# dashpay/agora-blsful

Hardware: NVIDIA B200
Metric: verified sigs/sec, 1M-batch G2Impl (higher is better)
Workload: dtype u32 limbs (381-bit modular integers)

## Files before the change

### agora-blsful_b200/csrc/blsgpu.cu

```cuda
#include <cuda_runtime.h>
#include <nvtx3/nvToolsExt.h>
#include <sys/random.h>

#include <algorithm>
#include <atomic>
#include <functional>
#include <cstdio>
#include <cstdlib>
#include <cstring>
#include <memory>
#include <mutex>
#include <string>
#include <unordered_map>
#include <thread>
#include <vector>

#include "../../include/blsgpu.h"
#include "kernels.cuh"

using namespace bls;

namespace {

thread_local std::string g_create_error;
// ... 347 lines not shown
  bool use_rlc = true, use_msm = false;
  int rbits = 0;
  std::vector<Level> lv;
  const PkA* d_pk = nullptr;
  const SigA *d_sig = nullptr, *d_h = nullptr;
  uint8_t* d_status = nullptr;
  Fp12* d_F = nullptr;
  SigJ *d_S = nullptr, *d_Sitem = nullptr, *d_msm_root = nullptr;
  RlcScalar* d_r = nullptr;
  Digest* d_root = nullptr;
  uint8_t* d_ok = nullptr;
  uint32_t* d_idx = nullptr;
  PkA* x_pk = nullptr;
  SigA* x_h = nullptr;
  uint8_t* x_pre = nullptr;
  M6Arg* x_args = nullptr;
  SLineRec* x_lines = nullptr;
  Fp12* x_T = nullptr;
  size_t x_cap = 0;
  M6Arg* big_args = nullptr;
  SLineRec* big_lines = nullptr;
  size_t big_items = 0;
  bool root_T_ready = false;
  const Fp12* rootF() const { return d_F + lv.back().off; }
  const SigJ* rootS() const { return use_msm ? d_msm_root : use_rlc ? d_S + lv.back().off : d_S; }
  bool big_rounds(size_t count) const { return count > PROBE_SMALL && big_items >= 6 * PROBE_SMALL; }
  size_t round_size(size_t count) const { return big_rounds(count) ? std::min(x_cap, big_items / 6) : PROBE_SMALL; }
};

size_t probe_cap(size_t leaves) { return std::max<size_t>(PROBE_SMALL, std::min<size_t>(leaves, 4096) + 16); }
template <class PkA, class SigA, class A>
void take_probe_scratch(A& a, Pipe<PkA, SigA>& P, size_t cap) {
  const size_t small = std::min(cap, PROBE_SMALL);
  P.x_cap = cap;
  P.d_ok = a.template take<uint8_t>(cap);
  P.d_idx = a.template take<uint32_t>(cap);
  P.x_pk = a.template take<PkA>(6 * cap);
  P.x_h = a.template take<SigA>(6 * cap);
  P.x_pre = a.template take<uint8_t>(6 * cap);
  P.x_T = a.template take<Fp12>(cap);
  P.x_args = a.template take<M6Arg>(6 * small);
  P.x_lines = a.template take<SLineRec>(6 * small * M6_LINE_RECS);
}
template <class PkA, class SigA>
size_t probe_scratch_bytes(size_t cap) {
  ArenaSize a;
  Pipe<PkA, SigA> P;
  take_probe_scratch(a, P, cap);
  return a.off;
}
template <class PkA, class SigA>
int set_probe_smem(blsgpu_ctx* ctx) {
  CK(cudaFuncSetAttribute(k_m6_lines<PkA, SigA>, cudaFuncAttributeMaxDynamicSharedMemorySize, M6_LINES_SMEM));
  CK(cudaFuncSetAttribute(k_m6_accum, cudaFuncAttributeMaxDynamicSharedMemorySize, M6_ACCUM_SMEM));
  CK(cudaFuncSetAttribute(k_final6, cudaFuncAttributeMaxDynamicSharedMemorySize, FE6_SMEM));
  return BLSGPU_OK;
}

template <class J>
int reduce_levels(blsgpu_ctx* ctx, const std::vector<Level>& lv, size_t first, Fp12* F, J* S) {
  for (size_t k = first; k + 1 < lv.size(); k++) {
    if (F) REDUCE_FP12(lv[k].cnt, (const Fp12*)(F + lv[k].off), lv[k + 1].cnt, F + lv[k + 1].off);
    if (S) REDUCE_JAC(J, lv[k].cnt, (const J*)(S + lv[k].off), lv[k + 1].cnt, S + lv[k + 1].off);
  }
  return BLSGPU_OK;
}

int seg_reduce(blsgpu_ctx* ctx, size_t n_out, const uint32_t* off, const Fp12* in, Fp12* out) {
  if (n_out <= REDUCE_WIDE_MAX)
    LAUNCH(k_seg_reduce_fp12_w, blocks_for(n_out * 16), TPB, n_out, off, in, out);
  else
    LAUNCH(k_seg_reduce_fp12, blocks_for(n_out), TPB, n_out, off, in, out);
  return BLSGPU_OK;
}
template <class J>
int seg_reduce(blsgpu_ctx* ctx, size_t n_out, const uint32_t* off, const J* in, J* out) {
  if (n_out <= REDUCE_WIDE_MAX)
    LAUNCH((k_seg_reduce_jac_w<J>), blocks_for(n_out * 16), TPB, n_out, off, in, out);
  else
    LAUNCH((k_seg_reduce_jac<J>), blocks_for(n_out), TPB, n_out, off, in, out);
  return BLSGPU_OK;
}
template <class T>
int seg_reduce_levels(blsgpu_ctx* ctx, const SegLevels& s, const uint32_t* d_off, T* nodes, T* top) {
  size_t in_off = 0, out_off = s.n[0], o = 0;
  for (size_t k = 1; k < s.n.size(); k++) {
    const size_t n_out = s.n[k];
    CKR(seg_reduce(ctx, n_out, d_off + o, (const T*)(nodes + in_off), k + 1 == s.n.size() ? top : nodes + out_off));
    o += n_out + 1;
    in_off = out_off;
    out_off += n_out;
  }
  return BLSGPU_OK;
}

int digest_root(blsgpu_ctx* ctx, size_t leaves, Digest* d_dig, Digest* d_root) {
  const std::vector<Level> ld = make_levels(leaves);
  for (size_t k = 0; k + 1 < ld.size(); k++)
    LAUNCH(k_digest_reduce, blocks_for(ld[k + 1].cnt), TPB, ld[k].cnt, d_dig + ld[k].off, ld[k + 1].cnt, d_dig + ld[k + 1].off);
  CK(cudaMemcpyAsync(d_root, d_dig + ld.back().off, sizeof(Digest), cudaMemcpyDeviceToDevice, ctx->stream));
  CK(cudaMemcpyAsync(d_root + 1, ctx->salt, 32, cudaMemcpyHostToDevice, ctx->stream));
  return BLSGPU_OK;
}

template <class PkA, class SigA>
int probe_miller(blsgpu_ctx* ctx, Pipe<PkA, SigA>& P, cudaStream_t stream, size_t cnt, M6Arg* args, SLineRec* lines) {
// ... 3160 lines not shown
```

### agora-blsful_b200/csrc/kernels.cuh

```cuda
#pragma once
#include <cuda_runtime.h>

#include "h2c.cuh"
#include "pairing.cuh"
#include "miller6.cuh"
#include "finalexp6.cuh"
#include "fr.cuh"

namespace bls {

template <class A>
struct PtInfo;
template <>
struct PtInfo<G1Aff> {
  static const int LEN = 48;
  typedef G1Jac Jac;
  typedef Fp F;
};
template <>
struct PtInfo<G2Aff> {
  static const int LEN = 96;
  typedef G2Jac Jac;
  typedef Fp2 F;
};
// ... 251 lines not shown
  size_t j = BLS_TID();
  if (j >= n_out) return;
  Sha256 s;
  sha256_init(s);
  for (int m = 0; m < 16; m++) {
    size_t idx = j + (size_t)m * n_out;
    if (idx < n_in) sha256_update(s, in[idx].b, 32);
  }
  Digest d;
  sha256_final(s, d.b);
  out[j] = d;
}
constexpr int RLC_MAX_WORDS = 4;
__device__ __forceinline__ void rlc_scalar(uint32_t k[RLC_MAX_WORDS], const Digest* root, size_t i, int rbits) {
  Sha256 s;
  sha256_init(s);
  sha256_update(s, root[0].b, 32);
  sha256_update(s, root[1].b, 32);
  uint8_t ib[8];
  for (int b = 0; b < 8; b++) ib[b] = (uint8_t)((uint64_t)i >> (8 * b));
  sha256_update(s, ib, 8);
  uint8_t d[32];
  sha256_final(s, d);
  uint32_t any = 0;
#pragma unroll
  for (int w = 0; w < RLC_MAX_WORDS; w++) {
    const uint32_t v = (uint32_t)d[4 * w] | ((uint32_t)d[4 * w + 1] << 8) | ((uint32_t)d[4 * w + 2] << 16) | ((uint32_t)d[4 * w + 3] << 24);
    k[w] = 32 * w < rbits ? v : 0u;
    any |= k[w];
  }
  if (any == 0) k[0] = 1;
}

__device__ __forceinline__ void miller_item(Fp12& f, const G1Aff& pk, const G2Aff& h, const uint32_t* k, bool scale) {
  MillerG1 mp;
  if (scale) {
    G1Jac pj;
    jac_mul_aff(pj, pk, k, 2);
    miller_prepare(mp, pj);
  } else {
    miller_prepare(mp, pk);
  }
  miller_loop(f, mp, h);
}
__device__ __forceinline__ void miller_item(Fp12& f, const G2Aff& pk, const G1Aff& h, const uint32_t* k, bool scale) {
  miller_item(f, h, pk, k, scale);
}
constexpr int M6_LINES_TPB = 128;
constexpr int M6_LINES_PAIRS = M6_LINES_TPB / 2;
constexpr int M6_LINES_SMEM = M6_NREG * M6_LINES_PAIRS * (int)sizeof(SFp2);
constexpr int M6_ITEMS_PER_BLOCK = 120;
constexpr int M6_ACCUM_SMEM = 4 * 30 * (int)sizeof(SAccRec);
constexpr size_t M6_LINE_RECS = (size_t)M6_STEPS * 3;

__device__ __forceinline__ const G1Aff& m6_g1(const G1Aff* pk, const G2Aff* h, size_t i) { return pk[i]; }
__device__ __forceinline__ const G1Aff& m6_g1(const G2Aff* pk, const G1Aff* h, size_t i) { return h[i]; }
__device__ __forceinline__ const G2Aff& m6_g2(const G1Aff* pk, const G2Aff* h, size_t i) { return h[i]; }
__device__ __forceinline__ const G2Aff& m6_g2(const G2Aff* pk, const G1Aff* h, size_t i) { return pk[i]; }

template <class PkA, class HA>
__global__ void __launch_bounds__(128, BLS_MIN_BLOCKS) k_m6_prep(size_t n, size_t base, const PkA* __restrict__ pk, const HA* __restrict__ h,
                                                 const uint8_t* __restrict__ pre, const Digest* __restrict__ root, int rbits,
                                                 M6Arg* __restrict__ args) {
  size_t c = BLS_TID();
  if (c >= n) return;
  const size_t i = base + c;
  if (pre[i] != ST_OK) return;
  G1Aff p = m6_g1(pk, h, i);
  MillerG1 mp;
  if (rbits) {
    uint32_t sc[RLC_MAX_WORDS];
    rlc_scalar(sc, root, i, rbits);
    G1Jac pj;
    jac_mul_aff_w4(pj, p, sc, rbits / 4);
    miller_prepare(mp, pj);
  } else {
    miller_prepare(mp, p);
  }
  M6Arg a;
  const G2Aff q = m6_g2(pk, h, i);
  m6_make_arg(a, mp, q);
  args[c] = a;
}

template <class PkA, class HA>
__global__ void __launch_bounds__(M6_LINES_TPB, 3) k_m6_lines(size_t n, size_t base, const M6Arg* __restrict__ args, const PkA* __restrict__ pk,
                                                             const HA* __restrict__ h, const uint8_t* __restrict__ pre, SLineRec* __restrict__ lines) {
  extern __shared__ __align__(16) uint8_t m6_smem[];
  const int hh = threadIdx.x & 1, pib = threadIdx.x >> 1;
  const size_t c = (size_t)blockIdx.x * M6_LINES_PAIRS + pib;
  const bool active = c < n && pre[base + (c < n ? c : 0)] == ST_OK;
  const size_t cc = active ? c : 0;
  const G2Aff& q = m6_g2(pk, h, base + cc);
  SopSpaces cx = m6_spaces_line(reinterpret_cast<SFp2*>(m6_smem) + pib, M6_LINES_PAIRS, args + cc, lines + cc * M6_LINE_RECS);
  if (active && hh == 0) {
    const G2Aff qv = q;
    m6_init_point(cx, qv);
  }
  __syncwarp();
  const uint64_t e = K_X_ABS;
#pragma unroll 1
  for (int i = 62; i >= 0; i--) {
#pragma unroll 1
    for (int pass = 0; pass < 1 + (int)((e >> i) & 1); pass++) {
      const M6Op* prog = pass == 0 ? K_M6_DBL : K_M6_ADD;
      const int nops = pass == 0 ? K_M6_DBL_N : K_M6_ADD_N;
#pragma unroll 1
      for (int o = 0; o < nops; o++) {
        const M6Op* op = prog + o;
        int32_t res[NL], other[NL];
        double vb = 0;
        if (active) vb = m6_op_compute(res, op, cx, hh);
        if (op->dst >= SOPX_LINE) {
#pragma unroll
          for (int j = 0; j < NL; j++) other[j] = __shfl_xor_sync(0xffffffffu, res[j], 1);
        }
        __syncwarp();
        if (active) m6_op_store(op, cx, hh, res, other, vb);
        __syncwarp();
      }
      cx.line += 3;
    }
  }
}

#ifndef M6_ACC_BLOCKS
#define M6_ACC_BLOCKS 3
#endif
__global__ void __launch_bounds__(128, M6_ACC_BLOCKS) k_m6_accum(size_t n, size_t base, const uint8_t* __restrict__ pre, const SLineRec* __restrict__ lines,
                                                     Fp12* __restrict__ out) {
  extern __shared__ __align__(16) uint8_t m6_smem[];
  const int warp = threadIdx.x >> 5, lane = threadIdx.x & 31;
  const int g = lane / 6, k = lane - 6 * g;
  const bool lane_on = g < 5;
  SAccRec* F = reinterpret_cast<SAccRec*>(m6_smem) + warp * 30 + 6 * (lane_on ? g : 0);
  const unsigned gsync = lane_on ? 63u << (6 * g) : 0xc0000000u;
  const size_t group = ((size_t)blockIdx.x * 4 + warp) * 5 + g;
  const size_t item = group * 6 + k;
  const bool active = lane_on && item < n && pre[base + item] == ST_OK;
  const unsigned ball = __ballot_sync(0xffffffffu, active);
  const unsigned gmask = lane_on ? (ball >> (6 * g)) & 63u : 0u;
  if (lane_on) {
    SFp2 init;
    if (k == 0) sfp2_one(init); else sfp2_zero(init);
    sacc_from_sfp2(F[k], init);
  }
  __syncwarp();
  const SLineRec* gl = lines + group * 6 * M6_LINE_RECS;
  const uint64_t e = K_X_ABS;
  int step = 0;
  if (gmask != 0) {
#pragma unroll 1
    for (int i = 62; i >= 0; i--) {
      if (i != 62) m6_sqr_lane(F + k, F, k, gsync);
      const int nst = 1 + (int)((e >> i) & 1);
#pragma unroll 1
      for (int st = 0; st < nst; st++, step++) {
#pragma unroll 1
        for (int j = 0; j < 6; j++) {
          {
            const int jn = j == 5 ? 0 : j + 1;
            const int sn = j == 5 ? step + 1 : step;
            if (k < 3 && sn < M6_STEPS) {
              const SLineRec* nx = gl + (size_t)jn * M6_LINE_RECS + 3 * sn + k;
              asm volatile("prefetch.global.L1 [%0];" ::"l"(nx));
              asm volatile("prefetch.global.L1 [%0];" ::"l"(reinterpret_cast<const uint8_t*>(nx) + 128));
            }
          }
          if ((gmask >> j) & 1u) m6_mul_line_lane(F + k, F, gl + (size_t)j * M6_LINE_RECS + 3 * step, k, gsync);
        }
      }
    }
  }
  __syncwarp();
  if (lane_on && group * 6 < n) m6_finish_lane(*fp12_coeff(out[base / 6 + group], k), F[k], k);
}

template <class SigA>
__global__ void __launch_bounds__(128, BLS_MIN_BLOCKS) k_scale_sig(size_t n, const SigA* __restrict__ sig, const uint8_t* __restrict__ pre,
                                                   const Digest* __restrict__ root, int rbits,
                                                   typename PtInfo<SigA>::Jac* __restrict__ out) {
  size_t i = BLS_TID();
  if (i >= n) return;
  typename PtInfo<SigA>::Jac s;
  if (pre[i] != ST_OK) {
    jac_set_inf(s);
  } else {
    uint32_t k[RLC_MAX_WORDS];
    rlc_scalar(k, root, i, rbits);
    SigA a = sig[i];
    jac_mul_aff(s, a, k, rbits / 32);
  }
  out[i] = s;
}

constexpr int MSM_CHUNK = 16;
struct RlcScalar {
  uint64_t lo, hi;
};
__device__ __forceinline__ uint32_t msm_digit(const RlcScalar& r, int c, int w) {
  const int bit = c * w;
  const uint64_t v = bit >= 64 ? r.hi >> (bit - 64) : bit == 0 ? r.lo : (r.lo >> bit) | (r.hi << (64 - bit));
  return (uint32_t)v & ((1u << c) - 1u);
}
__global__ void __launch_bounds__(128) k_msm_count(size_t n, const uint8_t* __restrict__ pre, const Digest* __restrict__ root, int rbits, int c,
                                                   int nwin, RlcScalar* __restrict__ r_out, uint32_t* __restrict__ counts) {
  size_t i = BLS_TID();
  if (i >= n) return;
  RlcScalar r = {0, 0};
  if (pre[i] == ST_OK) {
    uint32_t k[RLC_MAX_WORDS];
    rlc_scalar(k, root, i, rbits);
    r.lo = (uint64_t)k[0] | ((uint64_t)k[1] << 32);
    r.hi = (uint64_t)k[2] | ((uint64_t)k[3] << 32);
  }
  r_out[i] = r;
  for (int w = 0; w < nwin; w++) {
    const uint32_t d = msm_digit(r, c, w);
    if (d) atomicAdd(&counts[((size_t)w << c) + d], 1u);
  }
}
__global__ void __launch_bounds__(1024) k_msm_scan(int c, const uint32_t* __restrict__ counts, uint32_t* __restrict__ offsets,
                                                   uint32_t* __restrict__ cursor) {
// ... 1112 lines not shown
```

### agora-blsful_b200/csrc/miller6.cuh

```cuda
#pragma once
#include "pairing.cuh"
#include "sfp.cuh"

namespace bls {

constexpr int M6_GROUP = 6;

#define M6_S(ia, ib, xi, sh) {SOPX_F + ia, SOPX_F + ib, sh, 0, (xi) ? SOP_XI : 0, 0, 0, 0}
BLS_CONST SopTerm K_M6_SQR[6][4] = {
    {M6_S(0, 0, 0, 0), M6_S(1, 5, 1, 1), M6_S(2, 4, 1, 1), M6_S(3, 3, 1, 0)},
    {M6_S(0, 1, 0, 1), M6_S(2, 5, 1, 1), M6_S(3, 4, 1, 0), M6_S(3, 4, 1, 0)},
    {M6_S(0, 2, 0, 1), M6_S(1, 1, 0, 0), M6_S(3, 5, 1, 1), M6_S(4, 4, 1, 0)},
    {M6_S(0, 3, 0, 1), M6_S(1, 2, 0, 1), M6_S(4, 5, 1, 0), M6_S(4, 5, 1, 0)},
    {M6_S(0, 4, 0, 1), M6_S(1, 3, 0, 1), M6_S(2, 2, 0, 0), M6_S(5, 5, 1, 0)},
    {M6_S(0, 5, 0, 1), M6_S(1, 4, 0, 1), M6_S(2, 3, 0, 0), M6_S(2, 3, 0, 0)},
};
#undef M6_S
BLS_CONST SopTerm K_M6_MUL_LINE[3] = {
    {SOPX_FREL + 0, SOPX_JL + 0, 0, 0, 0, 0, 0, 0},
    {SOPX_FREL + 2, SOPX_JL + 1, 0, 0, SOP_XI_LT2, 0, 0, 0},
    {SOPX_FREL + 3, SOPX_JL + 2, 0, 0, SOP_XI_LT3, 0, 0, 0},
};

BLS_HD void m6_sqr_lane(SAccRec* out, const SAccRec* F, int k, unsigned sync_mask) { sopw(out, K_M6_SQR[k], 4, F, nullptr, k, sync_mask); }
BLS_HD void m6_mul_line_lane(SAccRec* out, const SAccRec* F, const SLineRec* line, int k, unsigned sync_mask) {
  sopw(out, K_M6_MUL_LINE, 3, F, line, k, sync_mask);
}

BLS_HD Fp2* fp12_coeff(Fp12& f, int k) {
  Fp6& h = (k & 1) ? f.c1 : f.c0;
  return (k >> 1) == 0 ? &h.c0 : (k >> 1) == 1 ? &h.c1 : &h.c2;
}

BLS_HD void m6_finish_lane(Fp2& out, const SAccRec& fa, int k) {
  SFp2 fk, t;
  sfp2_from_sacc(fk, fa);
  t = fk;
  if (k & 1) sfp2_neg(t, fk);
  Fp2 u;
  fp2_from_sfp2(u, t);
  fred(out, u);
}

enum : uint8_t {
  RX = 0, RY, RZ, RT0, RT1, RT2, RT3, RT4, RT5, RT6,
  M6_NREG,
  RPX = SOPX_P, RNPY = SOPX_P + 1, RPZ = SOPX_P + 2,
  RNQX = SOPX_P + 3, RQY = SOPX_P + 4,
  RL0 = SOPX_LINE, RL2 = SOPX_LINE + 1, RL3 = SOPX_LINE + 2,
  RNONE = SOPX_NONE
};
struct M6Op {
  uint8_t kind;
  uint8_t dst, nt, fp;
  SopTerm t[3];
  int8_t lx, ly, lz;
  uint8_t xr, yr, zr, lfl, pad;
};
#define M6_T(a, b) {a, b, 0, 0, 0, 0, 0, 0}
#define M6_TS(a, sha, b, shb, fl) {a, b, sha, shb, fl, 0, 0, 0}
#define M6_SQ(a) {a, a, 0, 0, SOP_SQR, 0, 0, 0}
#define M6_SQS(a, sha, shb, fl) {a, a, sha, shb, (fl) | SOP_SQR, 0, 0, 0}
#define M6_SOP1(dst, t0) {0, dst, 1, 0, {t0, t0, t0}, 0, 0, 0, RNONE, RNONE, RNONE, 0, 0}
#define M6_SOP2(dst, t0, t1) {0, dst, 2, 0, {t0, t1, t1}, 0, 0, 0, RNONE, RNONE, RNONE, 0, 0}
#define M6_SOP3(dst, t0, t1, t2) {0, dst, 3, 0, {t0, t1, t2}, 0, 0, 0, RNONE, RNONE, RNONE, 0, 0}
#define M6_SOPFP(dst, t0) {0, dst, 1, 1, {t0, t0, t0}, 0, 0, 0, RNONE, RNONE, RNONE, 0, 0}
#define M6_SOPFP2(dst, t0, t1) {0, dst, 2, 1, {t0, t1, t1}, 0, 0, 0, RNONE, RNONE, RNONE, 0, 0}
#define M6_LIN(dst, x, lx, fl, y, ly, z, lz) {1, dst, 0, 0, {M6_T(RNONE, RNONE), M6_T(RNONE, RNONE), M6_T(RNONE, RNONE)}, lx, ly, lz, x, y, z, fl, 0}
BLS_CONST M6Op K_M6_DBL[] = {
    M6_SOP1(RT0, M6_SQ(RY)),
    M6_SOP1(RT1, M6_SQ(RZ)),
    M6_SOP1(RT2, M6_SQ(RX)),
    M6_SOP1(RT3, M6_T(RX, RY)),
    M6_SOP1(RT4, M6_T(RY, RZ)),
    M6_LIN(RT1, RT1, 12, SOP_XI, RNONE, 0, RNONE, 0),
    M6_LIN(RT5, RT1, -3, 0, RT0, 1, RNONE, 0),
    M6_LIN(RT6, RT1, 3, 0, RT0, 1, RNONE, 0),
    M6_LIN(RT2, RT2, 3, 0, RNONE, 0, RNONE, 0),
    M6_SOP1(RX, M6_TS(RT3, 1, RT5, 0, 0)),
    M6_LIN(RT5, RT1, 1, 0, RT0, -1, RNONE, 0),
    M6_SOPFP(RL0, M6_T(RT5, RPZ)),
    M6_LIN(RT1, RT1, 2, 0, RNONE, 0, RNONE, 0),
    M6_SOP3(RY, M6_SQ(RT6), M6_SQS(RT1, 1, 0, SOP_NEG), M6_SQS(RT1, 0, 0, SOP_NEG)),
    M6_SOP1(RZ, M6_TS(RT0, 2, RT4, 1, 0)),
    M6_SOPFP(RL2, M6_T(RT2, RPX)),
    M6_SOPFP(RL3, M6_TS(RT4, 1, RNPY, 0, 0)),
};
BLS_CONST M6Op K_M6_ADD[] = {
    M6_SOP1(RT0, M6_T(RQY, RZ)),
    M6_SOP1(RT1, M6_TS(RNQX, 0, RZ, 0, SOP_NEG)),
    M6_LIN(RT0, RT0, 1, 0, RY, -1, RNONE, 0),
    M6_LIN(RT1, RT1, 1, 0, RX, -1, RNONE, 0),
    M6_SOP1(RT2, M6_SQ(RT1)),
    M6_SOP1(RT3, M6_T(RT1, RT2)),
    M6_SOP1(RT4, M6_T(RT2, RX)),
    M6_SOP2(RT2, M6_T(RT1, RQY), M6_T(RT0, RNQX)),
    M6_SOPFP(RL0, M6_T(RT2, RPZ)),
    M6_SOPFP(RL2, M6_T(RT0, RPX)),
    M6_SOPFP(RL3, M6_T(RT1, RNPY)),
    M6_SOP1(RT2, M6_SQ(RT0)),
    M6_SOP1(RT2, M6_T(RT2, RZ)),
    M6_LIN(RT2, RT2, 1, 0, RT3, -1, RT4, -2),
    M6_SOP1(RX, M6_T(RT1, RT2)),
    M6_SOP3(RY, M6_T(RT0, RT4), M6_TS(RT0, 0, RT2, 0, SOP_NEG), M6_TS(RT3, 0, RY, 0, SOP_NEG)),
    M6_SOP1(RZ, M6_T(RT3, RZ)),
};
#undef M6_T
#undef M6_TS
#undef M6_SQ
#undef M6_SQS
#undef M6_SOP1
#undef M6_SOP2
#undef M6_SOP3
#undef M6_SOPFP
#undef M6_SOPFP2
#undef M6_LIN
constexpr int K_M6_DBL_N = (int)(sizeof(K_M6_DBL) / sizeof(M6Op));
constexpr int K_M6_ADD_N = (int)(sizeof(K_M6_ADD) / sizeof(M6Op));

BLS_FN void m6_run(const M6Op* prog, int n, const SopSpaces& cx) {
#pragma unroll 1
  for (int i = 0; i < n; i++) {
    const M6Op* op = prog + i;
    const bool to_line = op->dst >= SOPX_LINE;
    SFp2* dst = to_line ? nullptr : sop_rec(cx, op->dst);
    if (op->kind == 0) {
      sop2f(dst, to_line ? cx.line + (op->dst - SOPX_LINE) : nullptr, op->t, op->nt, op->fp, cx);
    } else {
      sfp2_lin(*dst, sop_rec(cx, op->xr), op->lx, op->lfl, op->yr == RNONE ? nullptr : sop_rec(cx, op->yr), op->ly,
               op->zr == RNONE ? nullptr : sop_rec(cx, op->zr), op->lz);
    }
  }
}

BLS_HD double m6_op_compute(int32_t* res, const M6Op* op, const SopSpaces& cx, int h) {
  if (op->kind == 0) return sop1_compute(res, op->t, op->nt, op->fp, cx, h);
  return sfp2_lin_half(res, sop_rec(cx, op->xr), op->lx, op->lfl, op->yr == RNONE ? nullptr : sop_rec(cx, op->yr), op->ly,
                       op->zr == RNONE ? nullptr : sop_rec(cx, op->zr), op->lz, h);
}
// ... 39 lines not shown
```

### agora-blsful_b200/csrc/sfp.cuh

```cuda
#pragma once
#include "fp2.cuh"

#if !defined(SOP_KARATSUBA)
#define SOP_KARATSUBA 1
#endif

namespace bls {

struct alignas(16) SFp2 {
  int32_t w[2 * NL];
#if defined(BLS_TRACK)
  double vb;
  double lb;
#endif
};

struct alignas(16) SLineRec {
  int32_t w[48];
#if defined(BLS_TRACK)
  double vb, lb;
#endif
};
struct alignas(16) SAccRec {
  int32_t w[64];
// ... 98 lines not shown
    sb[i] = alu_add_s32(b[i], b[H + i]);
  }
#pragma unroll
  for (int i = 0; i < H; i++) {
#pragma unroll
    for (int j = 0; j < H; j++) T[H + i + j] += (uint64_t)((int64_t)sa[i] * (int64_t)sb[j]);
  }
#else
#pragma unroll
  for (int i = 0; i < NL; i++) {
#pragma unroll
    for (int j = 0; j < NL; j++) T[i + j] += (uint64_t)((int64_t)a[i] * (int64_t)b[j]);
  }
#endif
}

BLS_HD void sop_redc(int32_t* out, uint64_t* T) {
#pragma unroll
  for (int i = 0; i < NL; i++) {
    const uint32_t m = opaque32(((uint32_t)T[i] * K_PINV28) & M28);
#pragma unroll
    for (int j = 0; j < NL; j++) T[i + j] += (uint64_t)m * p28(j);
    T[i + 1] += (uint64_t)((int64_t)T[i] >> 28);
  }
  int64_t c = 0;
#pragma unroll
  for (int j = 0; j < NL - 1; j++) {
    c += (int64_t)T[NL + j];
    const int64_t t = c + (1 << 27);
    out[j] = (int32_t)((uint32_t)t & M28) - (1 << 27);
    c = t >> 28;
  }
  out[NL - 1] = (int32_t)(c + (int64_t)T[2 * NL - 1]);
}

struct alignas(16) SopKeep {
  uint64_t v[2 * NL];
};
BLS_HD void sop_keep_st(SopKeep& k, int i, uint64_t a, uint64_t b) {
#if defined(__CUDA_ARCH__)
  asm volatile("st.local.v2.u64 [%0], {%1, %2};" ::"l"(__cvta_generic_to_local(&k.v[2 * i])), "l"(a), "l"(b) : "memory");
#else
  k.v[2 * i] = a;
  k.v[2 * i + 1] = b;
#endif
}
BLS_HD void sop_keep_ld(const SopKeep& k, int i, uint64_t& a, uint64_t& b) {
#if defined(__CUDA_ARCH__)
  asm volatile("ld.local.v2.u64 {%0, %1}, [%2];" : "=l"(a), "=l"(b) : "l"(__cvta_generic_to_local(&k.v[2 * i])) : "memory");
#else
  a = k.v[2 * i];
  b = k.v[2 * i + 1];
#endif
}

struct SopPrep {
  int32_t m0, m1, n1, ng, sh;
};
BLS_HD SopPrep sop_prep(int half, int xi, int neg, int sh) {
  SopPrep p;
  const int p0 = half == 0, p1 = half == 1, p2 = half == 2;
  p.m0 = -((p1 ^ 1) | xi);
  p.m1 = -(((p2 & xi) ^ 1) & ((p0 & (xi ^ 1)) ^ 1));
  p.n1 = -(p0 & xi);
  p.ng = -neg;
  p.sh = sh + (p2 & xi);
  return p;
}
BLS_HD void sop_prep_apply(int32_t* x, const SopI4* r, const SopPrep& p) {
  int32_t t[2 * NL];
#pragma unroll
  for (int i = 0; i < 7; i++) {
    t[4 * i] = r[i].x;
    t[4 * i + 1] = r[i].y;
    t[4 * i + 2] = r[i].z;
    t[4 * i + 3] = r[i].w;
  }
#pragma unroll
  for (int i = 0; i < NL; i++) {
    const int32_t v = (int32_t)((uint32_t)((t[i] & p.m0) + (((t[NL + i] ^ p.n1) - p.n1) & p.m1)) << p.sh);
    x[i] = (v ^ p.ng) - p.ng;
  }
}
BLS_HD void sop_fetch(SopI4* r, const SFp2* p) {
  const SopI4* q = reinterpret_cast<const SopI4*>(p->w);
#pragma unroll
  for (int i = 0; i < 7; i++) r[i] = q[i];
}
BLS_HD int sop_term_xi(uint32_t fl, int lane_k) {
  return (int)((fl & SOP_XI) != 0) | ((int)((fl & SOP_XI_LT2) != 0) & (int)(lane_k < 2)) | ((int)((fl & SOP_XI_LT3) != 0) & (int)(lane_k < 3));
}

BLS_FN void sop2f(SFp2* dst, SLineRec* dst_line, const SopTerm* t, int nt, int fp_mode, const SopSpaces& cx_) {
  const SopSpaces cx = cx_;
  const int lane_k = cx.k;
  uint64_t T[2 * NL];
  SopKeep keep;
  int32_t res[2 * NL], x[NL], y[NL];
  SopI4 ra[7], rb[7];
#if defined(BLS_TRACK)
  double col = 0, vsum = 0;
  BLS_REQ(nt >= 1 && nt <= SOP_MAX_TERMS, "sop2f term count");
  for (int k = 0; k < nt; k++) {
    const SopTerm m = t[k];
    const SFp2 *pa = sop_rec(cx, m.a), *pb = sop_rec(cx, m.b);
    const double xi = sop_term_xi(m.fl, lane_k) ? 2.0 : 1.0;
// ... 97 lines not shown
    v.x = res[4 * i];
    v.y = res[4 * i + 1];
    v.z = res[4 * i + 2];
    v.w = res[4 * i + 3];
    q[i] = v;
  }
#if defined(BLS_TRACK)
  STRK(*dst, vsum / 2500.0 + 1.0, 134217728.0);
#endif
}

BLS_HD SopPrep sop1_prep_a(int sel, int xi, int neg, int sh) {
  SopPrep p;
  p.m0 = -((sel ^ 1) | xi);
  p.m1 = -(sel | xi);
  p.n1 = -(sel ^ 1);
  p.ng = -neg;
  p.sh = sh;
  return p;
}
BLS_HD SopPrep sop1_prep_b(int idx, int sh) {
  SopPrep p;
  p.m0 = -(idx ^ 1);
  p.m1 = -idx;
  p.n1 = 0;
  p.ng = 0;
  p.sh = sh;
  return p;
}
BLS_HD SopPrep sop1_prep_sqr_x(int h, int neg, int sh) {
  SopPrep p;
  p.m0 = -1;
  p.m1 = -(h ^ 1);
  p.n1 = 0;
  p.ng = -neg;
  p.sh = sh + h;
  return p;
}
BLS_HD SopPrep sop1_prep_sqr_y(int h, int sh) {
  SopPrep p;
  p.m0 = -(h ^ 1);
  p.m1 = -1;
  p.n1 = -(h ^ 1);
  p.ng = 0;
  p.sh = sh;
  return p;
}
BLS_HD double sop1_compute(int32_t* res, const SopTerm* t, int nt, int fp_mode, const SopSpaces& cx_, int h) {
  const SopSpaces cx = cx_;
  const int lane_k = cx.k;
  const SopTerm tm0 = t[0], tm1 = t[nt > 1 ? 1 : 0], tm2 = t[nt > 2 ? 2 : 0];
  uint64_t T[2 * NL];
  int32_t x[NL], y[NL];
  SopI4 ra[7], rb[7];
  double vout = 0;
#if defined(BLS_TRACK)
  double col = 0, vsum = 0;
  BLS_REQ(nt >= 1 && nt <= 3, "sop1 term count");
  for (int k = 0; k < nt; k++) {
    const SopTerm m = t[k];
    const SFp2 *pa = sop_rec(cx, m.a), *pb = sop_rec(cx, m.b);
    const double xi = sop_term_xi(m.fl, lane_k) ? 2.0 : 1.0;
    const double sq = (m.fl & SOP_SQR) ? 2.0 : 1.0;
    const double la = pa->lb * (double)(1 << m.sha) * xi, lb = pb->lb * (double)(1 << m.shb);
    BLS_REQ(la * sq < 1073741824.0 && lb * sq < 1073741824.0 && m.sha < 4 && m.shb < 4, "sop1 operand limb overflow");
    BLS_REQ(!(m.fl & SOP_SQR) || (m.a == m.b && !fp_mode && xi == 1.0), "sop1 square term");
    col += 14.0 * 2.0 * sq * la * lb;
    vsum += 2.0 * pa->vb * (double)(1 << m.sha) * xi * pb->vb * (double)(1 << m.shb);
  }
  {
    const double lim = 9223372036854775808.0 - 15.0 * 72057594037927936.0;
    BLS_REQ(col < lim, "sop1 column overflow");
    BLS_REQ(vsum / 2500.0 + 1.0 < 16.0, "sop1 result value bound");
  }
  vout = vsum / 2500.0 + 1.0;
#endif
#pragma unroll
  for (int i = 0; i < 2 * NL; i++) T[i] = 0;
  const int per = fp_mode ? 1 : 2;
  {
    const SopTerm m = tm0;
    sop_fetch(ra, sop_rec(cx, m.a));
    sop_fetch(rb, sop_rec(cx, m.b));
    if (m.fl & SOP_SQR) {
      sop_prep_apply(x, ra, sop1_prep_sqr_x(h, (m.fl & SOP_NEG) != 0, m.sha));
      sop_prep_apply(y, rb, sop1_prep_sqr_y(h, m.shb));
    } else {
      sop_prep_apply(x, ra, sop1_prep_a(fp_mode ? h : 0, sop_term_xi(m.fl, lane_k), (m.fl & SOP_NEG) != 0, m.sha));
      sop_prep_apply(y, rb, sop1_prep_b(fp_mode ? 0 : h, m.shb));
    }
  }
  int k = 0, q = 0;
  int nsteps = 0;
  nsteps += (tm0.fl & SOP_SQR) ? 1 : per;
  if (nt > 1) nsteps += (tm1.fl & SOP_SQR) ? 1 : per;
  if (nt > 2) nsteps += (tm2.fl & SOP_SQR) ? 1 : per;
#pragma unroll 1
  for (int s = 0; s < nsteps; s++) {
    const SopTerm cur = k == 0 ? tm0 : k == 1 ? tm1 : tm2;
    const int perk = (cur.fl & SOP_SQR) ? 1 : per;
    const int qw = (q + 1 == perk);
    const int q1 = qw ? 0 : q + 1;
    const int k1 = qw ? (k + 1 == nt ? 0 : k + 1) : k;
    const SopTerm m = k1 == 0 ? tm0 : k1 == 1 ? tm1 : tm2;
    sop_fetch(ra, sop_rec(cx, m.a));
    sop_fetch(rb, sop_rec(cx, m.b));
    sop_acc(T, x, y);
    const int sqr = (m.fl & SOP_SQR) != 0;
    const int sel = fp_mode ? h : q1;
    const int neg = (int)((m.fl & SOP_NEG) != 0) ^ ((fp_mode | sqr) ? 0 : (q1 & (h ^ 1)));
    const SopPrep pa = sqr ? sop1_prep_sqr_x(h, neg, m.sha) : sop1_prep_a(sel, sop_term_xi(m.fl, lane_k), neg, m.sha);
    const SopPrep pb = sqr ? sop1_prep_sqr_y(h, m.shb) : sop1_prep_b(fp_mode ? 0 : (q1 ^ h), m.shb);
    sop_prep_apply(x, ra, pa);
    sop_prep_apply(y, rb, pb);
    k = k1;
    q = q1;
  }
  T[2 * NL - 1] = 0;
  sop_redc(res, T);
  return vout;
}
BLS_HD void sop1_store_rec(SFp2* dst, const int32_t* res, int h, double vb) {
  int2* q = reinterpret_cast<int2*>(dst->w + NL * h);
#pragma unroll
  for (int i = 0; i < 7; i++) q[i] = make_int2(res[2 * i], res[2 * i + 1]);
  (void)vb;
  STRK(*dst, vb, 134217728.0);
}
BLS_HD void sop1_store_line(SLineRec* dst, const int32_t* res, const int32_t* other, int h, double vb) {
  SopI4* q = reinterpret_cast<SopI4*>(dst->w);
#pragma unroll
  for (int i = 0; i < 4; i++) {
    int32_t e[4], f[4];
#pragma unroll
    for (int z = 0; z < 4; z++) {
      const int j = 4 * i + z;
      e[z] = j >= NL ? 0 : res[j];
      f[z] = j >= NL ? 0 : res[j] + other[j];
    }
    SopI4 v, w;
    v.x = e[0]; v.y = e[1]; v.z = e[2]; v.w = e[3];
    w.x = f[0]; w.y = f[1]; w.z = f[2]; w.w = f[3];
    q[4 * h + i] = v;
    if (h == 0) q[8 + i] = w;
  }
  (void)vb;
  STRK(*dst, vb, 134217728.0);
}
BLS_HD double sfp2_lin_half(int32_t* res, const SFp2* x, int32_t sx, uint32_t flx, const SFp2* y, int32_t sy, const SFp2* z, int32_t sz, int h) {
  int64_t v[NL];
  double vb = 0;
  {
    int32_t t[2 * NL];
    sop_ld28(t, x);
#pragma unroll
    for (int i = 0; i < NL; i++) {
      const int32_t plain = t[NL * h + i];
      const int32_t mixed = h ? t[i] + t[NL + i] : t[i] - t[NL + i];
      v[i] = (int64_t)sx * (int64_t)((flx & SOP_XI) ? mixed : plain);
    }
#if defined(BLS_TRACK)
    vb = (sx < 0 ? -(double)sx : (double)sx) * x->vb * ((flx & SOP_XI) ? 2.0 : 1.0);
    BLS_REQ(x->lb < 1073741824.0, "sfp2_lin_half limb");
#endif
  }
  if (y != nullptr) {
    int32_t t[2 * NL];
    sop_ld28(t, y);
#pragma unroll
// ... 5 lines not shown
  if (z != nullptr) {
    int32_t t[2 * NL];
    sop_ld28(t, z);
#pragma unroll
    for (int i = 0; i < NL; i++) v[i] += (int64_t)sz * (int64_t)t[NL * h + i];
#if defined(BLS_TRACK)
    vb += (sz < 0 ? -(double)sz : (double)sz) * z->vb;
#endif
  }
  int64_t c = 0;
#pragma unroll
  for (int j = 0; j < NL - 1; j++) {
    c += v[j];
    const int64_t u = c + (1 << 27);
    res[j] = (int32_t)((uint32_t)u & M28) - (1 << 27);
    c = u >> 28;
  }
  res[NL - 1] = (int32_t)(c + v[NL - 1]);
#if defined(BLS_TRACK)
  BLS_REQ(vb < 1000.0, "sfp2_lin_half value bound");
#endif
  return vb;
}

BLS_HD const int32_t* sopw_run_a(const SAccRec* F, int lane_k, uint32_t i, int pass, int xi) {
  int jr = lane_k - ((int)i - SOPX_FREL);
  jr += jr < 0 ? 6 : 0;
  const int j = i >= SOPX_FREL ? jr : (int)i - SOPX_F;
  const int run = xi ? (pass == 0 ? 3 : pass == 1 ? 2 : 0) : pass;
  return F[j].w + 16 * run;
}
BLS_HD const int32_t* sopw_run_b(const SAccRec* F, const SLineRec* jl, uint32_t i, int pass) {
  const int is_jl = (i >= SOPX_JL) & (i < SOPX_FREL);
  const int32_t* base = is_jl ? jl[is_jl ? (int)i - SOPX_JL : 0].w : F[is_jl ? 0 : (int)i - SOPX_F].w;
  return base + 16 * pass;
}
BLS_HD void sopw_fetch(SopI4* r, const int32_t* p) {
  const SopI4* q = reinterpret_cast<const SopI4*>(p);
#pragma unroll
  for (int i = 0; i < 4; i++) r[i] = q[i];
}
BLS_HD void sopw_take(int32_t* x, const SopI4* r, int sh) {
  int32_t t[16];
#pragma unroll
  for (int i = 0; i < 4; i++) {
    t[4 * i] = r[i].x;
    t[4 * i + 1] = r[i].y;
    t[4 * i + 2] = r[i].z;
    t[4 * i + 3] = r[i].w;
  }
#pragma unroll
  for (int i = 0; i < NL; i++) x[i] = (int32_t)((uint32_t)t[i] << sh);
}
BLS_FN void sopw(SAccRec* dst, const SopTerm* t, int nt, const SAccRec* F, const SLineRec* jl, int lane_k, unsigned sync_mask) {
  uint64_t T[2 * NL];
  SopKeep keep;
  int32_t res[2 * NL], x[NL], y[NL];
  SopI4 ra[4], rb[4];
#if defined(BLS_TRACK)
  double col = 0, vsum = 0;
  BLS_REQ(nt >= 3 && nt <= 4, "sopw term count");
  for (int k = 0; k < nt; k++) {
    const SopTerm m = t[k];
    const double xi = sop_term_xi(m.fl, lane_k) ? 2.0 : 1.0;
    int jr = lane_k - ((int)m.a - SOPX_FREL);
    jr += jr < 0 ? 6 : 0;
    const SAccRec& A = F[m.a >= SOPX_FREL ? jr : (int)m.a - SOPX_F];
    const bool bj = m.b >= SOPX_JL && m.b < SOPX_FREL;
    const double lbb = bj ? jl[m.b - SOPX_JL].lb : F[m.b - SOPX_F].lb, vbb = bj ? jl[m.b - SOPX_JL].vb : F[m.b - SOPX_F].vb;
    const double la = A.lb * (double)(1 << m.sha) * xi;
    BLS_REQ(la < 1073741824.0 && lbb < 1073741824.0 && m.sha < 4 && m.shb == 0 && !(m.fl & SOP_NEG), "sopw operand");
    col += 14.0 * 2.0 * la * lbb;
    vsum += 2.0 * A.vb * (double)(1 << m.sha) * xi * vbb;
  }
  {
    const double lim = 9223372036854775808.0 - 15.0 * 72057594037927936.0;
    BLS_REQ(col < lim, "sopw column overflow");
    BLS_REQ(vsum / 2500.0 + 1.0 < 16.0, "sopw result value bound");
  }
#endif
#pragma unroll
  for (int i = 0; i < 2 * NL; i++) T[i] = 0;
#pragma unroll 1
  for (int pass = 0; pass < 3; pass++) {
#pragma unroll 1
    for (int k = 0; k < nt; k++) {
      const SopTerm m = t[k];
      const int xi = sop_term_xi(m.fl, lane_k);
      sopw_fetch(ra, sopw_run_a(F, lane_k, m.a, pass, xi));
      sopw_fetch(rb, sopw_run_b(F, jl, m.b, pass));
      sopw_take(x, ra, m.sha + (xi & (pass == 2)));
      sopw_take(y, rb, 0);
      sop_acc(T, x, y);
    }
    if (pass == 0) {
#pragma unroll
      for (int i = 0; i < NL; i++) {
        sop_keep_st(keep, i, T[2 * i], T[2 * i + 1]);
        T[2 * i] = T[2 * i + 1] = 0;
      }
    } else {
#pragma unroll
      for (int i = 0; i < NL; i++) {
        uint64_t u0, u1;
        sop_keep_ld(keep, i, u0, u1);
        const uint64_t v0 = T[2 * i], v1 = T[2 * i + 1];
        if (pass == 1) sop_keep_st(keep, i, u0 + v0, u1 + v1);
        T[2 * i] = pass == 1 ? u0 - v0 : v0 - u0;
        T[2 * i + 1] = pass == 1 ? u1 - v1 : v1 - u1;
      }
      T[2 * NL - 1] = 0;
      int32_t c[NL];
      sop_redc(c, T);
#pragma unroll
      for (int i = 0; i < NL; i++) {
        if (pass == 1) res[i] = c[i]; else res[NL + i] = c[i];
      }
#pragma unroll
      for (int i = 0; i < 2 * NL; i++) T[i] = 0;
    }
  }
#if defined(__CUDA_ARCH__)
  __syncwarp(sync_mask);
#else
  (void)sync_mask;
#endif
  SopI4* q = reinterpret_cast<SopI4*>(dst->w);
#pragma unroll
  for (int h = 0; h < 4; h++) {
#pragma unroll
    for (int i = 0; i < 4; i++) {
      int32_t e[4];
#pragma unroll
      for (int z = 0; z < 4; z++) {
        const int j = 4 * i + z;
        e[z] = j >= NL ? 0 : h == 0 ? res[j] : h == 1 ? res[NL + j] : h == 2 ? res[j] + res[NL + j] : res[j] - res[NL + j];
      }
      SopI4 v;
      v.x = e[0];
      v.y = e[1];
      v.z = e[2];
      v.w = e[3];
      q[4 * h + i] = v;
    }
  }
#if defined(BLS_TRACK)
  STRK(*dst, vsum / 2500.0 + 1.0, 134217728.0);
#endif
#if defined(__CUDA_ARCH__)
  __syncwarp(sync_mask);
#endif
}

BLS_FN void sfp2_lin(SFp2& r, const SFp2* x, int32_t sx, uint32_t flx, const SFp2* y, int32_t sy, const SFp2* z, int32_t sz) {
  int32_t t[2 * NL];
  int64_t v[2 * NL];
  sop_ld28(t, x);
  if (flx & SOP_XI) {
#pragma unroll
    for (int i = 0; i < NL; i++) {
      const int32_t d = t[i] - t[NL + i], e = t[i] + t[NL + i];
      v[i] = (int64_t)sx * (int64_t)d;
      v[NL + i] = (int64_t)sx * (int64_t)e;
    }
  } else {
#pragma unroll
    for (int i = 0; i < 2 * NL; i++) v[i] = (int64_t)sx * (int64_t)t[i];
  }
#if defined(BLS_TRACK)
  double vb = (sx < 0 ? -(double)sx : (double)sx) * x->vb * ((flx & SOP_XI) ? 2.0 : 1.0);
  BLS_REQ(x->lb < 1073741824.0, "sfp2_lin limb");
#endif
  if (y != nullptr) {
    sop_ld28(t, y);
#pragma unroll
    for (int i = 0; i < 2 * NL; i++) v[i] += (int64_t)sy * (int64_t)t[i];
#if defined(BLS_TRACK)
    vb += (sy < 0 ? -(double)sy : (double)sy) * y->vb;
#endif
  }
  if (z != nullptr) {
    sop_ld28(t, z);
#pragma unroll
    for (int i = 0; i < 2 * NL; i++) v[i] += (int64_t)sz * (int64_t)t[i];
#if defined(BLS_TRACK)
    vb += (sz < 0 ? -(double)sz : (double)sz) * z->vb;
#endif
  }
#pragma unroll
  for (int h = 0; h < 2; h++) {
    int64_t c = 0;
#pragma unroll
    for (int j = 0; j < NL - 1; j++) {
      c += v[h * NL + j];
      const int64_t u = c + (1 << 27);
      r.w[h * NL + j] = (int32_t)((uint32_t)u & M28) - (1 << 27);
      c = u >> 28;
    }
    r.w[h * NL + NL - 1] = (int32_t)(c + v[h * NL + NL - 1]);
  }
#if defined(BLS_TRACK)
  BLS_REQ(vb < 1000.0, "sfp2_lin value bound");
  STRK(r, vb, 134217728.0);
#endif
}
// ... 81 lines not shown
```

Baseline: 1.304 million.

## Cut register pressure in Miller line kernels to raise occupancy

```diff
diff --git a/agora-blsful_b200/csrc/blsgpu.cu b/agora-blsful_b200/csrc/blsgpu.cu
--- a/agora-blsful_b200/csrc/blsgpu.cu
+++ b/agora-blsful_b200/csrc/blsgpu.cu
@@ -423,6 +423,7 @@
 template <class PkA, class SigA>
 int set_probe_smem(blsgpu_ctx* ctx) {
   CK(cudaFuncSetAttribute(k_m6_lines<PkA, SigA>, cudaFuncAttributeMaxDynamicSharedMemorySize, M6_LINES_SMEM));
+  CK(cudaFuncSetAttribute(k_m6_lines<PkA, SigA>, cudaFuncAttributePreferredSharedMemoryCarveout, cudaSharedmemCarveoutMaxShared));
   CK(cudaFuncSetAttribute(k_m6_accum, cudaFuncAttributeMaxDynamicSharedMemorySize, M6_ACCUM_SMEM));
   CK(cudaFuncSetAttribute(k_final6, cudaFuncAttributeMaxDynamicSharedMemorySize, FE6_SMEM));
   return BLSGPU_OK;
diff --git a/agora-blsful_b200/csrc/kernels.cuh b/agora-blsful_b200/csrc/kernels.cuh
--- a/agora-blsful_b200/csrc/kernels.cuh
+++ b/agora-blsful_b200/csrc/kernels.cuh
@@ -327,6 +327,19 @@
 constexpr int M6_ITEMS_PER_BLOCK = 120;
 constexpr int M6_ACCUM_SMEM = 4 * 30 * (int)sizeof(SAccRec);
 constexpr size_t M6_LINE_RECS = (size_t)M6_STEPS * 3;
+constexpr uint64_t m6_add_steps(int half) {
+  uint64_t m[2] = {0, 0};
+  int s = 0;
+  for (int i = 62; i >= 0; i--) {
+    s++;
+    if ((K_X_ABS >> i) & 1) {
+      m[s >> 6] |= 1ull << (s & 63);
+      s++;
+    }
+  }
+  return m[half];
+}
+constexpr uint64_t M6_ADD_STEPS_LO = m6_add_steps(0), M6_ADD_STEPS_HI = m6_add_steps(1);
 
 __device__ __forceinline__ const G1Aff& m6_g1(const G1Aff* pk, const G2Aff* h, size_t i) { return pk[i]; }
 __device__ __forceinline__ const G1Aff& m6_g1(const G2Aff* pk, const G1Aff* h, size_t i) { return h[i]; }
@@ -359,7 +372,7 @@
 }
 
 template <class PkA, class HA>
-__global__ void __launch_bounds__(M6_LINES_TPB, 3) k_m6_lines(size_t n, size_t base, const M6Arg* __restrict__ args, const PkA* __restrict__ pk,
+__global__ void __launch_bounds__(M6_LINES_TPB, 4) k_m6_lines(size_t n, size_t base, const M6Arg* __restrict__ args, const PkA* __restrict__ pk,
                                                              const HA* __restrict__ h, const uint8_t* __restrict__ pre, SLineRec* __restrict__ lines) {
   extern __shared__ __align__(16) uint8_t m6_smem[];
   const int hh = threadIdx.x & 1, pib = threadIdx.x >> 1;
@@ -400,7 +413,7 @@
 }
 
 #ifndef M6_ACC_BLOCKS
-#define M6_ACC_BLOCKS 3
+#define M6_ACC_BLOCKS 4
 #endif
 __global__ void __launch_bounds__(128, M6_ACC_BLOCKS) k_m6_accum(size_t n, size_t base, const uint8_t* __restrict__ pre, const SLineRec* __restrict__ lines,
                                                      Fp12* __restrict__ out) {
@@ -422,28 +435,24 @@
   }
   __syncwarp();
   const SLineRec* gl = lines + group * 6 * M6_LINE_RECS;
-  const uint64_t e = K_X_ABS;
-  int step = 0;
   if (gmask != 0) {
 #pragma unroll 1
-    for (int i = 62; i >= 0; i--) {
-      if (i != 62) m6_sqr_lane(F + k, F, k, gsync);
-      const int nst = 1 + (int)((e >> i) & 1);
+    for (int step = 0; step < M6_STEPS; step++) {
+      const bool add = ((step < 64 ? M6_ADD_STEPS_LO >> step : M6_ADD_STEPS_HI >> (step - 64)) & 1u) != 0;
 #pragma unroll 1
-      for (int st = 0; st < nst; st++, step++) {
-#pragma unroll 1
-        for (int j = 0; j < 6; j++) {
-          {
-            const int jn = j == 5 ? 0 : j + 1;
-            const int sn = j == 5 ? step + 1 : step;
-            if (k < 3 && sn < M6_STEPS) {
-              const SLineRec* nx = gl + (size_t)jn * M6_LINE_RECS + 3 * sn + k;
-              asm volatile("prefetch.global.L1 [%0];" ::"l"(nx));
-              asm volatile("prefetch.global.L1 [%0];" ::"l"(reinterpret_cast<const uint8_t*>(nx) + 128));
-            }
+      for (int j = (step != 0 && !add) ? -1 : 0; j < 6; j++) {
+        const bool sq = j < 0;
+        if (!sq) {
+          const int jn = j == 5 ? 0 : j + 1;
+          const int sn = j == 5 ? step + 1 : step;
+          if (k < 3 && sn < M6_STEPS) {
+            const SLineRec* nx = gl + (size_t)jn * M6_LINE_RECS + 3 * sn + k;
+            asm volatile("prefetch.global.L1 [%0];" ::"l"(nx));
+            asm volatile("prefetch.global.L1 [%0];" ::"l"(reinterpret_cast<const uint8_t*>(nx) + 128));
           }
-          if ((gmask >> j) & 1u) m6_mul_line_lane(F + k, F, gl + (size_t)j * M6_LINE_RECS + 3 * step, k, gsync);
         }
+        if (sq || ((gmask >> j) & 1u))
+          sopw_body(F + k, sq ? K_M6_SQR[k] : K_M6_MUL_LINE, sq ? 4 : 3, F, gl + (size_t)(sq ? 0 : j) * M6_LINE_RECS + 3 * step, k, gsync);
       }
     }
   }
diff --git a/agora-blsful_b200/csrc/miller6.cuh b/agora-blsful_b200/csrc/miller6.cuh
--- a/agora-blsful_b200/csrc/miller6.cuh
+++ b/agora-blsful_b200/csrc/miller6.cuh
@@ -43,7 +43,7 @@
 }
 
 enum : uint8_t {
-  RX = 0, RY, RZ, RT0, RT1, RT2, RT3, RT4, RT5, RT6,
+  RX = 0, RY, RZ, RT0, RT1, RT2, RT3, RT4,
   M6_NREG,
   RPX = SOPX_P, RNPY = SOPX_P + 1, RPZ = SOPX_P + 2,
   RNQX = SOPX_P + 3, RQY = SOPX_P + 4,
@@ -68,23 +68,23 @@
 #define M6_SOPFP2(dst, t0, t1) {0, dst, 2, 1, {t0, t1, t1}, 0, 0, 0, RNONE, RNONE, RNONE, 0, 0}
 #define M6_LIN(dst, x, lx, fl, y, ly, z, lz) {1, dst, 0, 0, {M6_T(RNONE, RNONE), M6_T(RNONE, RNONE), M6_T(RNONE, RNONE)}, lx, ly, lz, x, y, z, fl, 0}
 BLS_CONST M6Op K_M6_DBL[] = {
-    M6_SOP1(RT0, M6_SQ(RY)),
-    M6_SOP1(RT1, M6_SQ(RZ)),
-    M6_SOP1(RT2, M6_SQ(RX)),
-    M6_SOP1(RT3, M6_T(RX, RY)),
-    M6_SOP1(RT4, M6_T(RY, RZ)),
-    M6_LIN(RT1, RT1, 12, SOP_XI, RNONE, 0, RNONE, 0),
-    M6_LIN(RT5, RT1, -3, 0, RT0, 1, RNONE, 0),
-    M6_LIN(RT6, RT1, 3, 0, RT0, 1, RNONE, 0),
-    M6_LIN(RT2, RT2, 3, 0, RNONE, 0, RNONE, 0),
-    M6_SOP1(RX, M6_TS(RT3, 1, RT5, 0, 0)),
-    M6_LIN(RT5, RT1, 1, 0, RT0, -1, RNONE, 0),
-    M6_SOPFP(RL0, M6_T(RT5, RPZ)),
-    M6_LIN(RT1, RT1, 2, 0, RNONE, 0, RNONE, 0),
-    M6_SOP3(RY, M6_SQ(RT6), M6_SQS(RT1, 1, 0, SOP_NEG), M6_SQS(RT1, 0, 0, SOP_NEG)),
-    M6_SOP1(RZ, M6_TS(RT0, 2, RT4, 1, 0)),
-    M6_SOPFP(RL2, M6_T(RT2, RPX)),
-    M6_SOPFP(RL3, M6_TS(RT4, 1, RNPY, 0, 0)),
+    M6_SOP1(RT0, M6_SQ(RX)),
+    M6_LIN(RT0, RT0, 3, 0, RNONE, 0, RNONE, 0),
+    M6_SOPFP(RL2, M6_T(RT0, RPX)),
+    M6_SOP1(RT0, M6_T(RX, RY)),
+    M6_SOP1(RT1, M6_T(RY, RZ)),
+    M6_SOP1(RT2, M6_SQ(RY)),
+    M6_SOP1(RT3, M6_SQ(RZ)),
+    M6_LIN(RT3, RT3, 12, SOP_XI, RNONE, 0, RNONE, 0),
+    M6_LIN(RT4, RT3, 1, 0, RT2, -1, RNONE, 0),
+    M6_SOPFP(RL0, M6_T(RT4, RPZ)),
+    M6_LIN(RT4, RT3, -3, 0, RT2, 1, RNONE, 0),
+    M6_SOP1(RX, M6_TS(RT0, 1, RT4, 0, 0)),
+    M6_LIN(RT4, RT3, 3, 0, RT2, 1, RNONE, 0),
+    M6_LIN(RT3, RT3, 2, 0, RNONE, 0, RNONE, 0),
+    M6_SOP3(RY, M6_SQ(RT4), M6_SQS(RT3, 1, 0, SOP_NEG), M6_SQS(RT3, 0, 0, SOP_NEG)),
+    M6_SOPFP(RL3, M6_TS(RT1, 1, RNPY, 0, 0)),
+    M6_SOP1(RZ, M6_TS(RT2, 2, RT1, 1, 0)),
 };
 BLS_CONST M6Op K_M6_ADD[] = {
     M6_SOP1(RT0, M6_T(RQY, RZ)),
diff --git a/agora-blsful_b200/csrc/sfp.cuh b/agora-blsful_b200/csrc/sfp.cuh
--- a/agora-blsful_b200/csrc/sfp.cuh
+++ b/agora-blsful_b200/csrc/sfp.cuh
@@ -174,6 +174,46 @@
   a = k.v[2 * i];
   b = k.v[2 * i + 1];
 #endif
+}
+struct alignas(16) SopRes {
+  int32_t v[2][16];
+};
+BLS_HD void sop_res_st(SopRes& r, int half, const int32_t* c) {
+#pragma unroll
+  for (int i = 0; i < 4; i++) {
+    const int32_t c0 = c[4 * i], c1 = c[4 * i + 1], c2 = 4 * i + 2 < NL ? c[4 * i + 2] : 0, c3 = 4 * i + 3 < NL ? c[4 * i + 3] : 0;
+#if defined(__CUDA_ARCH__)
+    asm volatile("st.local.v4.s32 [%0], {%1, %2, %3, %4};" ::"l"(__cvta_generic_to_local(&r.v[half][4 * i])), "r"(c0), "r"(c1), "r"(c2),
+                 "r"(c3) : "memory");
+#else
+    r.v[half][4 * i] = c0;
+    r.v[half][4 * i + 1] = c1;
+    r.v[half][4 * i + 2] = c2;
+    r.v[half][4 * i + 3] = c3;
+#endif
+  }
+}
+BLS_HD void sop_res_ld(const SopRes& r, int32_t* res) {
+#pragma unroll
+  for (int h = 0; h < 2; h++) {
+#pragma unroll
+    for (int i = 0; i < 4; i++) {
+      int32_t c0, c1, c2, c3;
+#if defined(__CUDA_ARCH__)
+      asm volatile("ld.local.v4.s32 {%0, %1, %2, %3}, [%4];" : "=r"(c0), "=r"(c1), "=r"(c2), "=r"(c3)
+                   : "l"(__cvta_generic_to_local(&r.v[h][4 * i])) : "memory");
+#else
+      c0 = r.v[h][4 * i];
+      c1 = r.v[h][4 * i + 1];
+      c2 = r.v[h][4 * i + 2];
+      c3 = r.v[h][4 * i + 3];
+#endif
+      const int32_t c[4] = {c0, c1, c2, c3};
+#pragma unroll
+      for (int z = 0; z < 4; z++)
+        if (4 * i + z < NL) res[NL * h + 4 * i + z] = c[z];
+    }
+  }
 }
 
 struct SopPrep {
@@ -377,7 +417,7 @@
   const SopTerm tm0 = t[0], tm1 = t[nt > 1 ? 1 : 0], tm2 = t[nt > 2 ? 2 : 0];
   uint64_t T[2 * NL];
   int32_t x[NL], y[NL];
-  SopI4 ra[7], rb[7];
+  SopI4 ra[7];
   double vout = 0;
 #if defined(BLS_TRACK)
   double col = 0, vsum = 0;
@@ -403,18 +443,6 @@
 #pragma unroll
   for (int i = 0; i < 2 * NL; i++) T[i] = 0;
   const int per = fp_mode ? 1 : 2;
-  {
-    const SopTerm m = tm0;
-    sop_fetch(ra, sop_rec(cx, m.a));
-    sop_fetch(rb, sop_rec(cx, m.b));
-    if (m.fl & SOP_SQR) {
-      sop_prep_apply(x, ra, sop1_prep_sqr_x(h, (m.fl & SOP_NEG) != 0, m.sha));
-      sop_prep_apply(y, rb, sop1_prep_sqr_y(h, m.shb));
-    } else {
-      sop_prep_apply(x, ra, sop1_prep_a(fp_mode ? h : 0, sop_term_xi(m.fl, lane_k), (m.fl & SOP_NEG) != 0, m.sha));
-      sop_prep_apply(y, rb, sop1_prep_b(fp_mode ? 0 : h, m.shb));
-    }
-  }
   int k = 0, q = 0;
   int nsteps = 0;
   nsteps += (tm0.fl & SOP_SQR) ? 1 : per;
@@ -422,24 +450,21 @@
   if (nt > 2) nsteps += (tm2.fl & SOP_SQR) ? 1 : per;
 #pragma unroll 1
   for (int s = 0; s < nsteps; s++) {
-    const SopTerm cur = k == 0 ? tm0 : k == 1 ? tm1 : tm2;
-    const int perk = (cur.fl & SOP_SQR) ? 1 : per;
+    const SopTerm m = k == 0 ? tm0 : k == 1 ? tm1 : tm2;
+    const int sqr = (m.fl & SOP_SQR) != 0;
+    const int perk = sqr ? 1 : per;
+    const int sel = fp_mode ? h : q;
+    const int neg = (int)((m.fl & SOP_NEG) != 0) ^ ((fp_mode | sqr) ? 0 : (q & (h ^ 1)));
+    const SopPrep pa = sqr ? sop1_prep_sqr_x(h, neg, m.sha) : sop1_prep_a(sel, sop_term_xi(m.fl, lane_k), neg, m.sha);
+    const SopPrep pb = sqr ? sop1_prep_sqr_y(h, m.shb) : sop1_prep_b(fp_mode ? 0 : (q ^ h), m.shb);
+    sop_fetch(ra, sop_rec(cx, m.a));
+    sop_prep_apply(x, ra, pa);
+    sop_fetch(ra, sop_rec(cx, m.b));
+    sop_prep_apply(y, ra, pb);
+    sop_acc(T, x, y);
     const int qw = (q + 1 == perk);
-    const int q1 = qw ? 0 : q + 1;
-    const int k1 = qw ? (k + 1 == nt ? 0 : k + 1) : k;
-    const SopTerm m = k1 == 0 ? tm0 : k1 == 1 ? tm1 : tm2;
-    sop_fetch(ra, sop_rec(cx, m.a));
-    sop_fetch(rb, sop_rec(cx, m.b));
-    sop_acc(T, x, y);
-    const int sqr = (m.fl & SOP_SQR) != 0;
-    const int sel = fp_mode ? h : q1;
-    const int neg = (int)((m.fl & SOP_NEG) != 0) ^ ((fp_mode | sqr) ? 0 : (q1 & (h ^ 1)));
-    const SopPrep pa = sqr ? sop1_prep_sqr_x(h, neg, m.sha) : sop1_prep_a(sel, sop_term_xi(m.fl, lane_k), neg, m.sha);
-    const SopPrep pb = sqr ? sop1_prep_sqr_y(h, m.shb) : sop1_prep_b(fp_mode ? 0 : (q1 ^ h), m.shb);
-    sop_prep_apply(x, ra, pa);
-    sop_prep_apply(y, rb, pb);
-    k = k1;
-    q = q1;
+    k = qw ? k + 1 : k;
+    q = qw ? 0 : q + 1;
   }
   T[2 * NL - 1] = 0;
   sop_redc(res, T);
@@ -551,11 +576,12 @@
 #pragma unroll
   for (int i = 0; i < NL; i++) x[i] = (int32_t)((uint32_t)t[i] << sh);
 }
-BLS_FN void sopw(SAccRec* dst, const SopTerm* t, int nt, const SAccRec* F, const SLineRec* jl, int lane_k, unsigned sync_mask) {
+BLS_HD void sopw_body(SAccRec* dst, const SopTerm* t, int nt, const SAccRec* F, const SLineRec* jl, int lane_k, unsigned sync_mask) {
   uint64_t T[2 * NL];
   SopKeep keep;
+  SopRes halves;
   int32_t res[2 * NL], x[NL], y[NL];
-  SopI4 ra[4], rb[4];
+  SopI4 ra[4];
 #if defined(BLS_TRACK)
   double col = 0, vsum = 0;
   BLS_REQ(nt >= 3 && nt <= 4, "sopw term count");
@@ -587,9 +613,9 @@
       const SopTerm m = t[k];
       const int xi = sop_term_xi(m.fl, lane_k);
       sopw_fetch(ra, sopw_run_a(F, lane_k, m.a, pass, xi));
-      sopw_fetch(rb, sopw_run_b(F, jl, m.b, pass));
       sopw_take(x, ra, m.sha + (xi & (pass == 2)));
-      sopw_take(y, rb, 0);
+      sopw_fetch(ra, sopw_run_b(F, jl, m.b, pass));
+      sopw_take(y, ra, 0);
       sop_acc(T, x, y);
     }
     if (pass == 0) {
@@ -611,14 +637,12 @@
       T[2 * NL - 1] = 0;
       int32_t c[NL];
       sop_redc(c, T);
-#pragma unroll
-      for (int i = 0; i < NL; i++) {
-        if (pass == 1) res[i] = c[i]; else res[NL + i] = c[i];
-      }
+      sop_res_st(halves, pass - 1, c);
 #pragma unroll
       for (int i = 0; i < 2 * NL; i++) T[i] = 0;
     }
   }
+  sop_res_ld(halves, res);
 #if defined(__CUDA_ARCH__)
   __syncwarp(sync_mask);
 #else
@@ -650,6 +674,9 @@
   __syncwarp(sync_mask);
 #endif
 }
+BLS_FN void sopw(SAccRec* dst, const SopTerm* t, int nt, const SAccRec* F, const SLineRec* jl, int lane_k, unsigned sync_mask) {
+  sopw_body(dst, t, nt, F, jl, lane_k, sync_mask);
+}
 
 BLS_FN void sfp2_lin(SFp2& r, const SFp2* x, int32_t sx, uint32_t flx, const SFp2* y, int32_t sy, const SFp2* z, int32_t sz) {
   int32_t t[2 * NL];
```

Result: faster. 1.337 million (median of 6 runs) (+2.5%).
